# Neptune-Crypto/twenty-first

Hardware: AMD Instinct MI355X
Metric: goldilocks_ntt_gfelts_per_s (higher is better)
Workload: dtype u64

## Files before the change

### include/tf_hip.h

```cpp
#ifndef TF_HIP_H
#define TF_HIP_H

#include <stddef.h>
#include <stdint.h>

#ifdef __cplusplus
extern "C" {
#endif

enum tf_status {
    TF_OK = 0,
    TF_ERR_TOO_FEW_LEAFS = 1,
    TF_ERR_INCORRECT_NUMBER_OF_LEAFS = 2,
    TF_ERR_TREE_TOO_HIGH = 3,
    TF_ERR_LEN_NOT_POWER_OF_TWO = 4,
    TF_ERR_LEN_TOO_LARGE = 5,
    TF_ERR_ORDER_NOT_ABOVE_DEGREE = 6,
    TF_ERR_NULL_POINTER = 7,
    TF_ERR_NO_DEVICE = 8,
    TF_ERR_HIP = 9,
    TF_ERR_OUT_OF_MEMORY = 10,
    TF_ERR_LEAF_INDEX_INVALID = 11,
    TF_ERR_INVERSE_OF_ZERO = 12,
    TF_ERR_BUFFER_TOO_SMALL = 13,
// ... 199 lines not shown
int tf_tip5_sponge_sample_indices_dev(uint64_t *d_states, size_t count, uint32_t upper_bound, size_t num_indices, uint32_t *d_out_u32,
                                      void *stream);

int tf_batch_inversion_bfe(const uint64_t *in, size_t n, uint64_t *out);
int tf_batch_inversion_xfe(const uint64_t *in, size_t n, uint64_t *out);
int tf_batch_inversion_bfe_dev(const uint64_t *d_in, size_t n, uint64_t *d_out, void *stream);
int tf_batch_inversion_xfe_dev(const uint64_t *d_in, size_t n, uint64_t *d_out, void *stream);
int tf_batch_inversion_bfe_dev_async(const uint64_t *d_in, size_t n, uint64_t *d_out, void *stream, int *d_status);
int tf_batch_inversion_xfe_dev_async(const uint64_t *d_in, size_t n, uint64_t *d_out, void *stream, int *d_status);
int tf_inverse_or_zero_bfe(const uint64_t *in, size_t n, uint64_t *out);
int tf_inverse_or_zero_xfe(const uint64_t *in, size_t n, uint64_t *out);
int tf_inverse_or_zero_bfe_dev(const uint64_t *d_in, size_t n, uint64_t *d_out, void *stream);
int tf_inverse_or_zero_xfe_dev(const uint64_t *d_in, size_t n, uint64_t *d_out, void *stream);

void tf_set_ntt_tile_bytes(size_t bytes);
size_t tf_get_ntt_tile_bytes(void);
void tf_set_ntt_pipe(int streams);
int tf_get_ntt_pipe(void);

void tf_set_ntt_min_passes(int passes);
void tf_set_ntt_small_launch(int mode);
void tf_set_ntt_two_pass(int mode);
void tf_set_ntt_latency_kernel(int mode);
int tf_ntt_launch_count(size_t n, size_t batch, int width);
int tf_ntt_plan(size_t n, int width, int* log2_radix_out);
double tf_debug_sclk_mhz(void);

#ifdef TF_AB_BUILD
void tf_set_ntt_nt(int mask);
void tf_set_ntt_chain(int tiles_per_workgroup);
int tf_debug_stamps(unsigned long long *host_out, size_t words);
#endif
int tf_debug_fill_random_dev(uint64_t *d_out, size_t count, uint64_t seed, uint64_t first_index, void *stream);

#ifdef __cplusplus
}
#endif
#endif
```

### twenty-first_amd/_lib.py

```python
from __future__ import annotations

import ctypes as C
import os
import subprocess

_HERE = os.path.dirname(os.path.abspath(__file__))
SO_PATH = os.environ.get("TF_HIP_LIBRARY") or os.path.join(_HERE, "libtf_hip.so")
HEADER = os.path.join(os.path.dirname(_HERE), "include", "tf_hip.h")

_u64p = C.POINTER(C.c_uint64)
_sz = C.c_size_t
_vp = C.c_void_p

SIGNATURES = {
    "tf_status_string": (C.c_char_p, [C.c_int]),
    "tf_last_error": (C.c_char_p, []),
    "tf_version": (C.c_int, []),
    "tf_source_hash": (C.c_char_p, []),
    "tf_device_count": (C.c_int, []),
    "tf_set_device": (C.c_int, [C.c_int]),
    "tf_get_device": (C.c_int, [C.POINTER(C.c_int)]),
    "tf_shard_range": (C.c_int, [_sz, C.c_int, C.c_int, C.POINTER(_sz), C.POINTER(_sz)]),
    "tf_merkle_multi_subtrees": (C.c_int, [_sz, _sz, C.c_int]),
    "tf_prepare_ntt": (C.c_int, [_sz, _sz, C.c_int, C.c_int]),
# ... 130 lines not shown
    "tf_tip5_sponge_pad_and_absorb_all_dev": (C.c_int, [_vp, _sz, _vp, _sz, _vp, _vp]),
    "tf_tip5_sponge_squeeze": (C.c_int, [_vp, _sz, _sz, _vp]),
    "tf_tip5_sponge_squeeze_dev": (C.c_int, [_vp, _sz, _sz, _vp, _vp]),
    "tf_tip5_sponge_sample_scalars": (C.c_int, [_vp, _sz, _sz, _vp]),
    "tf_tip5_sponge_sample_scalars_dev": (C.c_int, [_vp, _sz, _sz, _vp, _vp]),
    "tf_tip5_sponge_sample_indices": (C.c_int, [_vp, _sz, C.c_uint32, _sz, _vp]),
    "tf_tip5_sponge_sample_indices_dev": (C.c_int, [_vp, _sz, C.c_uint32, _sz, _vp, _vp]),
    "tf_merkle_verify_proofs": (C.c_int, [_vp, _sz, _vp, _vp, _vp, _vp, _vp, _vp, _vp]),
    "tf_merkle_verify_proofs_dev": (C.c_int, [_vp, _sz, _vp, _vp, _vp, _vp, _vp, _vp, _vp, _vp]),
    "tf_merkle_authentication_paths": (C.c_int, [_vp, _sz, _vp, _vp, _vp, _vp, _vp, _vp, _vp]),
    "tf_merkle_authentication_paths_dev": (C.c_int, [_vp, _sz, _vp, _vp, _vp, _vp, _vp, _vp, _vp, _vp]),
    "tf_ntt_launch_count": (C.c_int, [_sz, _sz, C.c_int]),
    "tf_ntt_plan": (C.c_int, [_sz, C.c_int, C.POINTER(C.c_int)]),
    "tf_batch_eval_plan": (C.c_int, [_sz, _sz, _sz, C.c_int]),
    "tf_poly_interpolate_bfe_dev_async": (C.c_int, [_vp, _vp, _sz, _sz, _vp, _vp, _vp]),
    "tf_poly_interpolate_xfe_dev_async": (C.c_int, [_vp, _vp, _sz, _sz, _vp, _vp, _vp]),
    "tf_poly_clean_divide_bfe_dev_async": (C.c_int, [_vp, _sz, _vp, _sz, _vp, _vp, _vp]),
    "tf_poly_clean_divide_many_bfe_dev_async": (C.c_int, [_vp, _sz, _sz, _vp, _sz, _vp, _vp, _vp]),
    "tf_zerofier_tree_new_bfe_dev_async": (C.c_int, [_vp, _sz, _vp, C.POINTER(C.c_void_p)]),
    "tf_zerofier_tree_new_xfe_dev_async": (C.c_int, [_vp, _sz, _vp, C.POINTER(C.c_void_p)]),
    "tf_zerofier_tree_interpolate_dev_async": (C.c_int, [_vp, _vp, _sz, _vp, _vp, _vp]),
    "tf_release_caches": (C.c_int, []),
    "tf_set_ntt_small_launch": (None, [C.c_int]),
    "tf_set_ntt_two_pass": (None, [C.c_int]),
    "tf_set_ntt_latency_kernel": (None, [C.c_int]),
    "tf_debug_sclk_mhz": (C.c_double, []),
    "tf_set_ntt_tile_bytes": (None, [_sz]),
    "tf_set_ntt_min_passes": (None, [C.c_int]),
    "tf_get_ntt_tile_bytes": (_sz, []),
    "tf_set_ntt_pipe": (None, [C.c_int]),
    "tf_get_ntt_pipe": (C.c_int, []),
    "tf_set_batch_eval_route": (None, [C.c_int]),
    "tf_debug_fill_random_dev": (C.c_int, [_vp, _sz, C.c_uint64, C.c_uint64, _vp]),
}


AB_SIGNATURES = {
    "tf_set_ntt_chain": (None, [C.c_int]),
    "tf_debug_stamps": (C.c_int, [_vp, _sz]),
    "tf_set_ntt_nt": (None, [C.c_int]),
}


def build(force: bool = False) -> str:
    csrc = os.path.join(_HERE, "csrc")
    args = ["make", "-C", csrc]
    if force:
        args.append("-B")
    args.append(f"-j{min(8, os.cpu_count() or 1)}")
    subprocess.check_call(args, stdout=subprocess.DEVNULL)
    return SO_PATH


_lib = None


def _load_hip_runtime() -> None:
    candidates = []
    try:
        import torch

        candidates.append(os.path.join(os.path.dirname(torch.__file__), "lib", "libamdhip64.so"))
    except Exception:
        pass
    candidates += ["/opt/rocm/lib/libamdhip64.so", "libamdhip64.so"]
    errors = []
# ... 38 lines not shown
```

### twenty-first_amd/csrc/aux_kernels.h

```cpp
#pragma once

#include "gl64.h"

namespace tfk {

using gl::u32;
using gl::u64;

__global__ void sclk_probe_kernel(unsigned long long* out) {
    const unsigned long long w0 = wall_clock64(), c0 = clock64();
    unsigned v = threadIdx.x;
    for (int i = 0; i < 200000; ++i) v = v * 1664525u + 1013904223u;
    const unsigned long long c1 = clock64(), w1 = wall_clock64();
    if (threadIdx.x == 0) {
        out[0] = c1 - c0 + (v == 0xdeadbeefu);
        out[1] = w1 - w0;
    }
}

__global__ void __launch_bounds__(256) fill_random_kernel(u64* out, unsigned long long count, u64 seed, unsigned long long first) {
    const unsigned long long stride = (unsigned long long)gridDim.x * blockDim.x;
    for (unsigned long long i = (unsigned long long)blockIdx.x * blockDim.x + threadIdx.x; i < count; i += stride) {
        u64 z = (seed ^ (first + i)) + 0x9e3779b97f4a7c15ULL;
        z = (z ^ (z >> 30)) * 0xbf58476d1ce4e5b9ULL;
        z = (z ^ (z >> 27)) * 0x94d049bb133111ebULL;
        z ^= z >> 31;
        if (z >= gl::P) z -= gl::P;
        out[i] = gl::mont_mul(z, gl::R2);
    }
}

}
```

### twenty-first_amd/csrc/gl64.h

```cpp
#pragma once

#include <stdint.h>

#if defined(__HIPCC__)
#include <hip/hip_runtime.h>
#define GL_HD __host__ __device__ __forceinline__
#else
#define GL_HD inline
#endif

namespace gl {

typedef uint64_t u64;
typedef uint32_t u32;

constexpr u64 P = 0xffffffff00000001ULL;
constexpr u64 EPS = 0xffffffffULL;
constexpr u64 R2 = 0xfffffffe00000001ULL;
constexpr u64 ONE = 0xffffffffULL;

GL_HD u64 add(u64 a, u64 b) {
    u64 s = a + b;
    bool c = s < a;
    u64 t = s + EPS;
// ... 416 lines not shown
    static_assert(K > 0 && K < 32, "");
    const u64 lo = x << K;
    const u32 hi = (u32)(x >> (64 - K));
    const u64 t = (u64)hi * 0xffffffffu + lo;
    const bool c = t < lo;
    const u64 u = t + EPS;
    const bool c2 = u < t;
    return (c | c2) ? u : t;
}

template <int S>
GL_HD u64 shl_monty(u64 x) {
    static_assert(S >= 0 && S < 64, "");
#if defined(__HIP_DEVICE_COMPILE__)
    const u32 x0 = (u32)x, x1 = (u32)(x >> 32);
    u32 l0, l1, h0, h1;
    if constexpr (S == 0) {
        l0 = x0, l1 = x1, h0 = 0, h1 = 0;
    } else if constexpr (S < 32) {
        l0 = x0 << S, l1 = __builtin_amdgcn_alignbit(x1, x0, 32 - S), h0 = x1 >> (32 - S), h1 = 0;
    } else if constexpr (S == 32) {
        l0 = 0, l1 = x0, h0 = x1, h1 = 0;
    } else {
        l0 = 0, l1 = x0 << (S - 32), h0 = __builtin_amdgcn_alignbit(x1, x0, 64 - S), h1 = x1 >> (64 - S);
    }
    return montyred(((u64)l1 << 32) | l0, ((u64)h1 << 32) | h0);
#else
    const u64 lo = x << S;
    const u64 hi = S ? (x >> ((64 - S) & 63)) : 0;
    return montyred(lo, hi);
#endif
}

template <int E>
struct Pow2Mul {
    static constexpr int e96 = ((E % 192) + 192) % 192 % 96;
    static constexpr bool high = (((E % 192) + 192) % 192) >= 96;
    static constexpr bool via_monty = e96 >= 32;
    static constexpr bool negate = high != via_monty;
    static GL_HD u64 apply(u64 x) {
        if constexpr (e96 == 0) {
            return x;
        } else if constexpr (e96 < 32) {
            return shl_fold<e96>(x);
        } else {
            return shl_monty<e96 - 32>(x);
        }
    }
};

template <int K>
GL_HD u64 mul_pow2(u64 x) {
    const u64 v = Pow2Mul<K>::apply(x);
    if constexpr (Pow2Mul<K>::negate) return neg(v);
    return v;
}

}
```

### twenty-first_amd/csrc/ntt_kernels.h

```cpp
#pragma once

#include <type_traits>

#include "gl64.h"
#include "ntt_args.h"
#include "ntt_network.h"

namespace tfk {

using gl::u32;
using gl::u64;

struct NttPassArgs {
    const u64* in;
    u64* out;
    const u64* inner_tw;
    const u64* post_tw;
    const u64* pre_scale;
    long long n_out;
    const u64* in2;
    const u64* post_scale;
    long long js_i0, js_i1, js_i2, js_c, js_k;
    long long n_coeffs;
    long long ps_i1;
// ... 1093 lines not shown
            for (int i = 0; i < 8; ++i) wb[i] = tw_load(8 + i);
        }
        mul_store(0, wa);
#pragma unroll
        for (int i = 0; i < 8; ++i) wa[i] = tw_load(16 + i);
        __builtin_amdgcn_sched_barrier(0);
        mul_store(8, wb);
#pragma unroll
        for (int i = 0; i < 8; ++i) wb[i] = tw_load(24 + i);
        __builtin_amdgcn_sched_barrier(0);
        mul_store(16, wa);
        __builtin_amdgcn_sched_barrier(0);
        mul_store(24, wb);
    }
}

struct NttBlockArgs {
    const u64* in;
    u64* out;
    const u64* tw1;
    const u64* tw2;
    const u64* pre_scale;
    const u64* post_scale;
    long long n_coeffs;
    long long in_bs, out_bs;
    long long total_transforms;
    const u64* in2;
    long long n_out;
    int L;
};

template <int LOGP3, bool INV, int SCALE = 0>
__global__ void __launch_bounds__(512, 4) ntt_block_kernel(const NttBlockArgs A) {
    constexpr int P3 = 1 << LOGP3, N = 1024 << LOGP3, REST = 32 << LOGP3, T = 16 >> LOGP3;
    constexpr int PS1 = 1056 + 32 / P3;
    constexpr int KS2 = 32 * P3 + 1;
    extern __shared__ __attribute__((aligned(16))) u64 lds[];
    const int t = threadIdx.x;
    const long long tr0 = (long long)blockIdx.x * T;
    const int nt = (int)min((long long)T, A.total_transforms - tr0);
    u64 x[32];
    const int trA = t / REST, rest = t - trA * REST;
    const bool actA = trA < nt;
    const int es = A.L;
    {
        const long long ltA = tr0 + trA, slA = ltA / es;
        const u64* src = A.in + slA * A.in_bs + (ltA - slA * es) + (long long)rest * es;
        const long long lim = (SCALE != 1 || A.n_coeffs < 0) ? (long long)N : A.n_coeffs;
#pragma unroll
        for (int q = 0; q < 32; ++q) x[q] = (actA && (SCALE != 1 || brev5(q) * REST + rest < lim)) ? src[(long long)brev5(q) * REST * es] : 0;
        if (SCALE == 3) {
            const u64* src2 = A.in2 + (tr0 + trA) * A.in_bs + rest;
#pragma unroll
            for (int q0 = 0; q0 < 32; q0 += 8) {
                u64 w[8];
#pragma unroll
                for (int i = 0; i < 8; ++i) w[i] = actA ? src2[(long long)brev5(q0 + i) * REST] : 0;
#pragma unroll
                for (int i = 0; i < 8; i += 4) mul4_inplace(x, q0 + i, w[i], w[i + 1], w[i + 2], w[i + 3]);
            }
        }
        if (SCALE == 1 && A.pre_scale) {
            const u64* ps = A.pre_scale + rest;
#pragma unroll
            for (int q0 = 0; q0 < 32; q0 += 8) {
                u64 w[8];
#pragma unroll
                for (int i = 0; i < 8; ++i) {
                    const long long j = brev5(q0 + i) * REST + rest;
                    w[i] = ps[j < lim ? brev5(q0 + i) * REST : -rest];
                }
#pragma unroll
                for (int i = 0; i < 8; i += 4) mul4_inplace(x, q0 + i, w[i], w[i + 1], w[i + 2], w[i + 3]);
            }
        }
    }
    dit_half<INV, 0, true>(x);
    dit_half<INV, 16, true>(x);
    dit_level<INV, 5, true>(x);
    {
        const u64* tw = A.tw1 + rest;
#pragma unroll
        for (int q = 4; q < 32; q += 4) mul4_inplace(x, q, tw[q * REST], tw[(q + 1) * REST], tw[(q + 2) * REST], tw[(q + 3) * REST]);
        gl::mont_mul2(x[2], tw[2 * REST], x[3], tw[3 * REST], x[2], x[3]);
        x[1] = gl::mont_mul(x[1], tw[REST]);
#if TF_LAZY
        x[0] = gl::add(x[0], 0);
#endif
    }
    const int j2A = rest >> LOGP3, j3A = rest & (P3 - 1);
    const int pairA = trA * P3 + j3A;
    const int tb = (LOGP3 == 4) ? ((t & ~0x108) | ((t & 8) << 5) | ((t >> 5) & 8)) : t;
    const int trB = tb / REST, j3B = (tb >> 5) & (P3 - 1), k1B = tb & 31;
    const int pairB = trB * P3 + j3B;
#pragma unroll 1
    for (int r = 0; r < 2; ++r) {
        if (r) __syncthreads();
        if ((pairA >> 3) == r) {
            u64* wr = lds + (pairA & 7) * PS1 + j2A;
#pragma unroll
            for (int q = 0; q < 32; ++q) wr[q * 33] = x[q];
        }
        __syncthreads();
        if ((pairB >> 3) == r) {
            const u64* rd = lds + (pairB & 7) * PS1 + k1B * 33;
#pragma unroll
            for (int q = 0; q < 32; ++q) x[q] = rd[brev5(q)];
        }
    }
    dit_half<INV, 0, true>(x);
    dit_half<INV, 16, true>(x);
    dit_level<INV, 5, true>(x);
    {
        const u64* tw = A.tw2 + j3B;
#pragma unroll
        for (int q = 0; q < 32; q += 4) mul4_inplace(x, q, tw[q * P3], tw[(q + 1) * P3], tw[(q + 2) * P3], tw[(q + 3) * P3]);
    }
    const int trC = trB, sC = j3B, k1C = k1B;
    __syncthreads();
#pragma unroll 1
    for (int r = 0; r < 2; ++r) {
        if (r) __syncthreads();
        if ((k1B >> 4) == r) {
            u64* wr = lds + (trB * 16 + (k1B & 15)) * KS2 + j3B;
#pragma unroll
            for (int q = 0; q < 32; ++q) wr[q * P3] = x[q];
        }
        __syncthreads();
        if ((k1C >> 4) == r) {
            const u64* rd = lds + (trC * 16 + (k1C & 15)) * KS2 + sC * (32 / P3) * P3;
#pragma unroll
            for (int q = 0; q < 32; ++q) {
                const int grp = q >> LOGP3, rr = q & (P3 - 1);
                const int j3 = (int)(__brev((unsigned)rr) >> (32 - LOGP3));
                x[q] = rd[grp * P3 + j3];
            }
        }
    }
    if constexpr (LOGP3 >= 1) dit_level<INV, 1>(x);
    if constexpr (LOGP3 >= 2) dit_level<INV, 2>(x);
    if constexpr (LOGP3 >= 3) dit_level<INV, 3>(x);
    if constexpr (LOGP3 >= 4) dit_level<INV, 4>(x);
    if (trC < nt) {
        const long long ltC = tr0 + trC, slC = ltC / es;
        u64* dst = A.out + slC * A.out_bs + (ltC - slC * es) + (long long)k1C * es;
// ... 329 lines not shown
```

### twenty-first_amd/csrc/ntt_network.h

```cpp
#pragma once

#include "gl64.h"

namespace tfk {

using gl::u32;
using gl::u64;

template <bool INV, int LVL, int J>
struct TwExp {
    static constexpr int fwd = ((39 << (6 - LVL)) * J) % 192;
    static constexpr int value = INV ? (192 - fwd) % 192 : fwd;
};

#ifndef TF_ASM_BFLY
#define TF_ASM_BFLY 1
#endif
#ifndef TF_LDS_TW
#define TF_LDS_TW 1
#endif
constexpr int kLdsTwStride = 34;
constexpr int kR1024Nc = 16, kR1024Cpr = 8, kR1024Rounds = 2, kR1024S1 = 264;
constexpr int kL1024S1 = 273, kL1024CS = 34;
constexpr int kL1024ExchangeWords = ((31 * kL1024S1 + 7 * kL1024CS + 32 + 1) / 2) * 2;
#ifndef TF_LAZY
#define TF_LAZY 1
#endif

template <bool INV, int LVL, int I>
struct Bf {
    static constexpr int H = 1 << (LVL - 1);
    static constexpr int j = I % H;
    static constexpr int ia = (I / H) * 2 * H + j;
    static constexpr int ib = ia + H;
    static constexpr int E = TwExp<INV, LVL, j>::value;
    static constexpr bool neg = gl::Pow2Mul<E>::negate;
};

template <int E, bool LAZY_IN>
__device__ __forceinline__ u64 tw_operand(u64 b) {
    if constexpr (E % 192 == 0) {
        if constexpr (LAZY_IN) return gl::add(b, 0);
        return b;
    } else {
        return gl::Pow2Mul<E>::apply(b);
    }
}

template <bool INV, int LVL, int I, bool LAZY>
__device__ __forceinline__ void butterfly_pair(u64 (&x)[32]) {
    using B0 = Bf<INV, LVL, I>;
    using B1 = Bf<INV, LVL, I + 1>;
    const u64 v0 = tw_operand<B0::E, LAZY && (LVL > 1)>(x[B0::ib]);
    const u64 v1 = tw_operand<B1::E, LAZY && (LVL > 1)>(x[B1::ib]);
    u64 s0, d0, s1, d1;
    if constexpr (LAZY) gl::add_sub_lazy2(x[B0::ia], v0, x[B1::ia], v1, s0, d0, s1, d1);
    else gl::add_sub2(x[B0::ia], v0, x[B1::ia], v1, s0, d0, s1, d1);
    x[B0::ia] = B0::neg ? d0 : s0;
    x[B0::ib] = B0::neg ? s0 : d0;
    x[B1::ia] = B1::neg ? d1 : s1;
    x[B1::ib] = B1::neg ? s1 : d1;
}

template <int E>
__device__ __forceinline__ void butterfly_pow2(u64& a, u64& b) {
    const u64 v = gl::Pow2Mul<E>::apply(b);
#if TF_ASM_BFLY
    if constexpr (!gl::Pow2Mul<E>::negate) gl::add_sub(a, v, a, b);
    else gl::add_sub(a, v, b, a);
    return;
#endif
    if constexpr (!gl::Pow2Mul<E>::negate) {
        const u64 s = gl::add(a, v);
        b = gl::sub(a, v);
        a = s;
    } else {
        const u64 s = gl::sub(a, v);
        b = gl::add(a, v);
        a = s;
    }
}

template <bool INV, int LVL, int I, int END, bool LAZY>
struct DitRange {
    static __device__ __forceinline__ void run(u64 (&x)[32]) {
#if TF_ASM_BFLY
        butterfly_pair<INV, LVL, I, LAZY>(x);
#else
        butterfly_pow2<Bf<INV, LVL, I>::E>(x[Bf<INV, LVL, I>::ia], x[Bf<INV, LVL, I>::ib]);
        butterfly_pow2<Bf<INV, LVL, I + 1>::E>(x[Bf<INV, LVL, I + 1>::ia], x[Bf<INV, LVL, I + 1>::ib]);
#endif
        if constexpr (I + 2 < END) DitRange<INV, LVL, I + 2, END, LAZY>::run(x);
    }
};
template <bool INV, int LVL, bool LAZY = false>
__device__ __forceinline__ void dit_level(u64 (&x)[32]) { DitRange<INV, LVL, 0, 16, LAZY && TF_LAZY>::run(x); }

template <bool INV, int FIRST, bool LAZY = false>
__device__ __forceinline__ void dit_half(u64 (&x)[32]) {
    DitRange<INV, 1, FIRST / 2, FIRST / 2 + 8, LAZY && TF_LAZY>::run(x);
    DitRange<INV, 2, FIRST / 2, FIRST / 2 + 8, LAZY && TF_LAZY>::run(x);
    DitRange<INV, 3, FIRST / 2, FIRST / 2 + 8, LAZY && TF_LAZY>::run(x);
    DitRange<INV, 4, FIRST / 2, FIRST / 2 + 8, LAZY && TF_LAZY>::run(x);
}

__device__ __forceinline__ void mul4_inplace(u64 (&x)[32], int q0, u64 w0, u64 w1, u64 w2, u64 w3) {
    const u64 a4[4] = {x[q0], x[q0 + 1], x[q0 + 2], x[q0 + 3]}, b4[4] = {w0, w1, w2, w3};
    u64 r4[4];
    gl::mont_mul4(a4, b4, r4);
    x[q0] = r4[0], x[q0 + 1] = r4[1], x[q0 + 2] = r4[2], x[q0 + 3] = r4[3];
}

}
```

### twenty-first_amd/csrc/tf_abi.hip

```cpp
#include "tf_internal.h"
#include "aux_kernels.h"

#include <functional>

namespace tfi {

struct DevBuf {
    u64* p = nullptr;
    hipStream_t s;
    explicit DevBuf(hipStream_t st) : s(st) {}
    int alloc(size_t words) {
        if (words == 0) return TF_OK;
        hipError_t e = pool_malloc_async(reinterpret_cast<void**>(&p), words * sizeof(u64), s);
        if (e != hipSuccess) return hip_fail(e, "hipMallocAsync", __FILE__, __LINE__);
        return TF_OK;
    }
    ~DevBuf() {
        if (p) (void)hipFreeAsync(p, s);
    }
};

int h2d(u64* d, const u64* h, size_t words, hipStream_t s) {
    if (!words) return TF_OK;
    HIPCHK(hipMemcpyAsync(d, h, words * sizeof(u64), hipMemcpyHostToDevice, s));
    HIPCHK(hipStreamSynchronize(s));
    return TF_OK;
}

struct HostStreams {
    hipStream_t s[kMaxDevices] = {};
    ~HostStreams() {
        for (int d = 0; d < kMaxDevices; ++d)
            if (s[d]) (void)hipStreamDestroy(s[d]);
    }
};
hipStream_t host_stream() {
// ... 71 lines not shown
int merkle_proofs_host(const uint32_t* heights, size_t n, const uint64_t* loff, const uint64_t* idx, const uint64_t* dig, const uint64_t* aoff,
                       const uint64_t* auth, const uint64_t* roots, int* statuses, uint64_t* paths_out, bool paths) {
    if (n == 0) return TF_OK;
    if (!heights || !loff || !aoff || !statuses) return TF_ERR_NULL_POINTER;
    size_t path_words = 0;
    for (size_t p = 0; p < n; ++p) {
        if (loff[p + 1] < loff[p] || aoff[p + 1] < aoff[p]) return TF_ERR_INVALID_ARGUMENT;
        if (heights[p] < 64) path_words += (loff[p + 1] - loff[p]) * heights[p];
    }
    const size_t nk = loff[n] - loff[0], na = aoff[n] - aoff[0];
    if ((nk && (!idx || !dig)) || (na && !auth) || (!paths && !roots) || (paths && path_words && !paths_out)) return TF_ERR_NULL_POINTER;
    DeviceCtx* ctx = nullptr;
    TRY(current_ctx(&ctx));
    hipStream_t s = host_stream();
    DevBuf di(s), dd(s), da(s), dr(s), dst(s), dp(s);
    TRY(di.alloc(nk));
    TRY(dd.alloc(5 * nk));
    TRY(da.alloc(5 * na));
    TRY(dr.alloc(paths ? 0 : 5 * n));
    TRY(dst.alloc((n + 1) / 2));
    TRY(dp.alloc(paths ? 5 * path_words : 0));
    if (nk) {
        TRY(h2d(di.p, idx + loff[0], nk, s));
        TRY(h2d(dd.p, dig + 5 * loff[0], 5 * nk, s));
    }
    if (na) TRY(h2d(da.p, auth + 5 * aoff[0], 5 * na, s));
    if (!paths) TRY(h2d(dr.p, roots, 5 * n, s));
    TRY(merkle_proofs_dev(heights, n, loff, di.p, dd.p, aoff, da.p, dr.p, reinterpret_cast<int*>(dst.p), dp.p, paths, loff[0], aoff[0], s));
    HIPCHK(hipMemcpyAsync(statuses, dst.p, n * sizeof(int), hipMemcpyDeviceToHost, s));
    if (paths) TRY(d2h(paths_out, dp.p, 5 * path_words, s));
    return sync(s);
}

}

using namespace tfi;


extern "C" {

const char* tf_status_string(int status) {
    switch (status) {
        case TF_OK: return "TF_OK";
        case TF_ERR_TOO_FEW_LEAFS: return "TF_ERR_TOO_FEW_LEAFS";
        case TF_ERR_INCORRECT_NUMBER_OF_LEAFS: return "TF_ERR_INCORRECT_NUMBER_OF_LEAFS";
        case TF_ERR_TREE_TOO_HIGH: return "TF_ERR_TREE_TOO_HIGH";
        case TF_ERR_LEN_NOT_POWER_OF_TWO: return "TF_ERR_LEN_NOT_POWER_OF_TWO";
        case TF_ERR_LEN_TOO_LARGE: return "TF_ERR_LEN_TOO_LARGE";
        case TF_ERR_ORDER_NOT_ABOVE_DEGREE: return "TF_ERR_ORDER_NOT_ABOVE_DEGREE";
        case TF_ERR_NULL_POINTER: return "TF_ERR_NULL_POINTER";
        case TF_ERR_NO_DEVICE: return "TF_ERR_NO_DEVICE";
        case TF_ERR_HIP: return "TF_ERR_HIP";
        case TF_ERR_OUT_OF_MEMORY: return "TF_ERR_OUT_OF_MEMORY";
        case TF_ERR_LEAF_INDEX_INVALID: return "TF_ERR_LEAF_INDEX_INVALID";
        case TF_ERR_INVERSE_OF_ZERO: return "TF_ERR_INVERSE_OF_ZERO";
        case TF_ERR_BUFFER_TOO_SMALL: return "TF_ERR_BUFFER_TOO_SMALL";
        case TF_ERR_EMPTY_DOMAIN: return "TF_ERR_EMPTY_DOMAIN";
        case TF_ERR_DIVISION_BY_ZERO: return "TF_ERR_DIVISION_BY_ZERO";
        case TF_ERR_DIVISION_NOT_CLEAN: return "TF_ERR_DIVISION_NOT_CLEAN";
        case TF_ERR_INVALID_ARGUMENT: return "TF_ERR_INVALID_ARGUMENT";
        case TF_ERR_INTERNAL: return "TF_ERR_INTERNAL";
        case TF_ERR_AUTH_STRUCTURE_LENGTH_MISMATCH: return "TF_ERR_AUTH_STRUCTURE_LENGTH_MISMATCH";
        case TF_ERR_REPEATED_LEAF_DIGEST_MISMATCH: return "TF_ERR_REPEATED_LEAF_DIGEST_MISMATCH";
        case TF_ERR_ROOT_MISMATCH: return "TF_ERR_ROOT_MISMATCH";
        case TF_ERR_MMR_LEAF_INDEX_OUT_OF_RANGE: return "TF_ERR_MMR_LEAF_INDEX_OUT_OF_RANGE";
        case TF_ERR_MMR_PEAK_COUNT_MISMATCH: return "TF_ERR_MMR_PEAK_COUNT_MISMATCH";
// ... 48 lines not shown
}
int tf_get_ntt_pipe(void) {
    read_env();
    return g_pipe.load(std::memory_order_relaxed);
}

double tf_debug_sclk_mhz(void) {
    int dev = 0, wall_khz = 0;
    if (hipGetDevice(&dev) != hipSuccess) return -1.0;
    if (hipDeviceGetAttribute(&wall_khz, hipDeviceAttributeWallClockRate, dev) != hipSuccess || wall_khz <= 0) wall_khz = 100000;
    unsigned long long* d = nullptr;
    if (hipMalloc(reinterpret_cast<void**>(&d), 2 * sizeof(unsigned long long)) != hipSuccess) return -1.0;
    hipLaunchKernelGGL(tfk::sclk_probe_kernel, dim3(1), dim3(64), 0, hipStream_t(0), d);
    unsigned long long h[2] = {0, 0};
    const hipError_t e = hipMemcpy(h, d, sizeof(h), hipMemcpyDeviceToHost);
    (void)hipFree(d);
    if (e != hipSuccess || h[1] == 0) return -1.0;
    return (double)h[0] / (double)h[1] * (double)wall_khz / 1000.0;
}

int tf_debug_fill_random_dev(uint64_t* d_out, size_t count, uint64_t seed, uint64_t first_index, void* stream) try {
    if (count == 0) return TF_OK;
    if (!d_out) return TF_ERR_NULL_POINTER;
    DeviceCtx* ctx = nullptr;
    int rc = current_ctx(&ctx);
    if (rc) return rc;
    const unsigned blocks = (unsigned)std::min<size_t>((count + 255) / 256, size_t(1) << 20);
    hipLaunchKernelGGL(tfk::fill_random_kernel, dim3(blocks), dim3(256), 0, static_cast<hipStream_t>(stream), d_out,
                       (unsigned long long)count, (u64)seed, (unsigned long long)first_index);
    HIPCHK(hipGetLastError());
    return TF_OK;
} TF_ABI_CATCH

#ifdef TF_AB_BUILD
int tf_debug_stamps(unsigned long long* host_out, size_t words) try {
    if (!g_dbg_buf) {
        if (hipMalloc(reinterpret_cast<void**>(&g_dbg_buf), 4096 * 8 * 6 * 8) != hipSuccess) return TF_ERR_HIP;
        (void)hipMemset(g_dbg_buf, 0, 4096 * 8 * 6 * 8);
    }
    if (host_out && words) {
        if (hipDeviceSynchronize() != hipSuccess) return TF_ERR_HIP;
        if (hipMemcpy(host_out, g_dbg_buf, std::min<size_t>(words, 4096 * 8 * 6) * 8, hipMemcpyDeviceToHost) != hipSuccess) return TF_ERR_HIP;
    }
    return TF_OK;
} TF_ABI_CATCH
#endif

void tf_set_ntt_min_passes(int passes) { g_min_passes.store(passes, std::memory_order_relaxed); }
#ifdef TF_AB_BUILD
void tf_set_ntt_chain(int tiles_per_workgroup) { g_chain.store(std::max(0, tiles_per_workgroup), std::memory_order_relaxed); }
#endif
void tf_set_ntt_latency_kernel(int mode) { g_lat_mode.store(mode < 0 ? -1 : (mode ? 1 : 0), std::memory_order_relaxed); }
void tf_set_ntt_two_pass(int mode) { g_pre2_mode.store(mode < 0 ? -1 : (mode > 3 ? 1 : mode), std::memory_order_relaxed); }
void tf_set_ntt_small_launch(int mode) { g_small_launch_mode.store(mode < 0 ? -1 : (mode ? 1 : 0), std::memory_order_relaxed); }
int tf_batch_eval_plan(size_t n_coeffs, size_t n_points, size_t batch, int width) {
    if (width != 1 && width != 3) return 0;
    return tree_route(n_coeffs, n_points, batch, width) ? 2 : 1;
}
int tf_ntt_plan(size_t n, int width, int* log2_radix_out) {
    if (check_len(n) || n <= 1 || (width != 1 && width != 3) || !log2_radix_out) return 0;
    const int log_n = ilog2(n);
    for (int i = 0; i < 4; ++i) log2_radix_out[i] = 0;
    static const bool no_block = ab_env("TF_NTT_NO_BLOCK") != nullptr;
    static const bool no_xfe_block = ab_env("TF_NTT_NO_XFE_BLOCK") != nullptr;
    if (log_n <= 10 || (log_n <= (width == 1 ? 14 : (no_xfe_block ? 10 : 12)) && !no_block && g_min_passes.load(std::memory_order_relaxed) == 0)) {
        log2_radix_out[0] = log_n;
// ... 776 lines not shown
```

### twenty-first_amd/device.py

```python
from __future__ import annotations

import ctypes as C

from . import _lib


def _chk(rc, where):
    from . import _check

    _check(rc, where)


def _t(t, name="tensor"):
    import torch

    if not isinstance(t, torch.Tensor) or not t.is_cuda or not t.is_contiguous() or t.dtype not in (torch.int64, torch.uint64):
        raise TypeError(f"{name} must be a contiguous CUDA int64/uint64 tensor of raw Montgomery words")
    return t


def _stream(stream):
    import torch

    s = stream if stream is not None else torch.cuda.current_stream()
    return C.c_void_p(s.cuda_stream)


def _p(t):
    return C.c_void_p(t.data_ptr())


def _need(cond: bool, what: str) -> None:
    if not cond:
        raise ValueError(what)


def _width(width: int) -> int:
    _need(width in (1, 3), "width must be 1 (BFieldElement) or 3 (XFieldElement)")
    return width


def fill_random(out, seed: int, first_index: int = 0, stream=None) -> None:
    out = _t(out, "out")
    _chk(_lib.lib().tf_debug_fill_random_dev(_p(out), out.numel(), C.c_uint64(seed & (2 ** 64 - 1)), C.c_uint64(first_index),
                                             _stream(stream)), "fill_random")


def ntt_(x, n: int, batch: int = 1, width: int = 1, inverse: bool = False, stream=None) -> None:
    x = _t(x, "x")
    _width(width)
    if x.numel() != n * batch * width:
        raise ValueError("tensor size is not batch * n * width")
    fn = _lib.lib().tf_ntt_bfe_dev if width == 1 else _lib.lib().tf_ntt_xfe_dev
    _chk(fn(_p(x), n, batch, int(inverse), _stream(stream)), "intt" if inverse else "ntt")


def coset_evaluate(coeffs, n_coeffs: int, offset_raw: int, out, order: int, batch: int = 1, width: int = 1, stream=None) -> None:
    coeffs, out = _t(coeffs, "coeffs"), _t(out, "out")
    _width(width)
    if coeffs.numel() != n_coeffs * batch * width or out.numel() != order * batch * width:
        raise ValueError("buffer sizes do not match n_coeffs/order/batch/width")
    fn = _lib.lib().tf_coset_eval_bfe_dev if width == 1 else _lib.lib().tf_coset_eval_xfe_dev
    _chk(fn(_p(coeffs), n_coeffs, C.c_uint64(offset_raw), _p(out), order, batch, _stream(stream)), "fast_coset_evaluate")


def tip5_permute_(states, stream=None) -> None:
    states = _t(states, "states")
    _need(states.numel() % 16 == 0, "states must hold 16 words per Tip5 state")
    _chk(_lib.lib().tf_tip5_permute_dev(_p(states), states.numel() // 16, _stream(stream)), "Tip5::permutation")


def tip5_trace_(states, trace, stream=None) -> None:
    states, trace = _t(states, "states"), _t(trace, "trace")
    _need(states.numel() % 16 == 0 and trace.numel() == 6 * states.numel(), "trace must hold 6 x 16 words per Tip5 state")
    _chk(_lib.lib().tf_tip5_trace_dev(_p(states), _p(trace), states.numel() // 16, _stream(stream)), "Tip5::trace")


def tip5_hash_pairs(inp, out, stream=None) -> None:
# ... 496 lines not shown
```

Baseline: 146.0.

## Group power-of-two twiddle butterflies by class and use inline asm reduction

Adds hand-written GCN inline assembly for the shift-and-reduce multiplications by powers of two in Goldilocks, batched 2 or 4 wide so independent carry chains interleave without nops. The radix-32 butterfly network now reorders butterflies within a level by exponent class so same-class twiddles can share one asm block. The aim is to cut VALU instruction count and dependency stalls in the block NTT kernel. It also adds a debug kernel and ABI entry to test mul_pow2. The risks are register pressure, and inline asm that may block compiler scheduling or hide a subtle carry bug.

```diff
diff --git a/include/tf_hip.h b/include/tf_hip.h
--- a/include/tf_hip.h
+++ b/include/tf_hip.h
@@ -255,6 +255,7 @@
 int tf_debug_stamps(unsigned long long *host_out, size_t words);
 #endif
 int tf_debug_fill_random_dev(uint64_t *d_out, size_t count, uint64_t seed, uint64_t first_index, void *stream);
+int tf_debug_mul_pow2_dev(uint64_t *d_x, size_t count, int e, void *stream);
 
 #ifdef __cplusplus
 }
diff --git a/twenty-first_amd/_lib.py b/twenty-first_amd/_lib.py
--- a/twenty-first_amd/_lib.py
+++ b/twenty-first_amd/_lib.py
@@ -186,6 +186,7 @@
     "tf_get_ntt_pipe": (C.c_int, []),
     "tf_set_batch_eval_route": (None, [C.c_int]),
     "tf_debug_fill_random_dev": (C.c_int, [_vp, _sz, C.c_uint64, C.c_uint64, _vp]),
+    "tf_debug_mul_pow2_dev": (C.c_int, [_vp, _sz, C.c_int, _vp]),
 }
 
 
diff --git a/twenty-first_amd/csrc/aux_kernels.h b/twenty-first_amd/csrc/aux_kernels.h
--- a/twenty-first_amd/csrc/aux_kernels.h
+++ b/twenty-first_amd/csrc/aux_kernels.h
@@ -30,4 +30,29 @@
     }
 }
 
+template <int E>
+__global__ void __launch_bounds__(256) mul_pow2_kernel(u64* x, unsigned long long count) {
+    const unsigned long long base = ((unsigned long long)blockIdx.x * blockDim.x + threadIdx.x) * 6;
+    u64 v4[4], v2[2];
+#pragma unroll
+    for (int i = 0; i < 4; ++i) v4[i] = base + i < count ? x[base + i] : 0;
+#pragma unroll
+    for (int i = 0; i < 2; ++i) v2[i] = base + 4 + i < count ? x[base + 4 + i] : 0;
+    if constexpr (gl::Pow2Mul<E>::cls == 0) {
+#pragma unroll
+        for (int i = 0; i < 4; ++i) v4[i] = gl::add(v4[i], 0);
+#pragma unroll
+        for (int i = 0; i < 2; ++i) v2[i] = gl::add(v2[i], 0);
+    } else {
+        gl::pow2_mul_block<E, E, E, E>(v4);
+        gl::pow2_mul_block<E, E>(v2);
+    }
+#pragma unroll
+    for (int i = 0; i < 4; ++i)
+        if (base + i < count) x[base + i] = gl::Pow2Mul<E>::negate ? gl::neg(v4[i]) : v4[i];
+#pragma unroll
+    for (int i = 0; i < 2; ++i)
+        if (base + 4 + i < count) x[base + 4 + i] = gl::Pow2Mul<E>::negate ? gl::neg(v2[i]) : v2[i];
 }
+
+}
diff --git a/twenty-first_amd/csrc/gl64.h b/twenty-first_amd/csrc/gl64.h
--- a/twenty-first_amd/csrc/gl64.h
+++ b/twenty-first_amd/csrc/gl64.h
@@ -472,22 +472,151 @@
 #endif
 }
 
+#ifndef TF_ASM_POW2
+#define TF_ASM_POW2 1
+#endif
+
+#if defined(__HIPCC__)
+template <int K>
+__device__ __forceinline__ u64 shl_fold_asm(u64 x) {
+    static_assert(K > 0 && K < 32, "");
+    const u64 lo = x << K;
+    const u32 hi = (u32)(x >> 32) >> (32 - K);
+    u64 t, c, ge, n;
+    asm("v_mad_u64_u32 %0, %1, %2, -1, %3" : "=v"(t), "=s"(c) : "v"(hi), "v"(lo));
+    u32 r0, r1;
+    asm("v_cmp_lt_u64_e64 %[ge], %[pm1], %[t]\n\t"
+        "s_or_b64 %[c], %[c], %[ge]\n\t"
+        "v_subbrev_co_u32_e64 %[r0], %[n], 0, %[t0], %[c]\n\t"
+        "s_andn2_b64 %[c], %[c], %[n]\n\t"
+        "v_addc_co_u32_e64 %[r1], %[n], 0, %[t1], %[c]"
+        : [r0] "=&v"(r0), [r1] "=v"(r1), [c] "+s"(c), [n] "=&s"(n), [ge] "=&s"(ge)
+        : [pm1] "s"(P - 1), [t] "v"(t), [t0] "v"((u32)t), [t1] "v"((u32)(t >> 32))
+        : "scc");
+    return ((u64)r1 << 32) | r0;
+}
+
+__device__ __forceinline__ u64 canonical_asm(u64 x) {
+    u32 r0, r1;
+    u64 c, n;
+    asm("v_cmp_lt_u64_e64 %[n], %[pm1], %[x]\n\t"
+        "s_mov_b64 %[c], %[n]\n\t"
+        "v_subbrev_co_u32_e64 %[r0], %[n], 0, %[x0], %[c]\n\t"
+        "s_andn2_b64 %[c], %[c], %[n]\n\t"
+        "v_addc_co_u32_e64 %[r1], %[n], 0, %[x1], %[c]"
+        : [r0] "=&v"(r0), [r1] "=v"(r1), [c] "=&s"(c), [n] "=&s"(n)
+        : [pm1] "s"(P - 1), [x] "v"(x), [x0] "v"((u32)x), [x1] "v"((u32)(x >> 32))
+        : "scc");
+    return ((u64)r1 << 32) | r0;
+}
+
+#define TF_P2_RR1(S) S(a)
+#define TF_P2_RR2(S) S(a) S(b)
+#define TF_P2_RR4(S) S(a) S(b) S(c) S(d)
+#define TF_P2_GAP1 "s_nop 1\n\t"
+#define TF_P2_GAP2 "s_nop 0\n\t"
+#define TF_P2_GAP4
+#define TF_P2B_1(X) "v_add_co_u32_e64 %[u" #X "], %[c" #X "], %[u" #X "], %[w" #X "]\n\t"
+#define TF_P2B_2(X) "v_subb_co_u32_e64 %[w" #X "], %[c" #X "], %[w" #X "], %[u" #X "], %[c" #X "]\n\t"
+#define TF_P2B_3(X) "v_subbrev_co_u32_e64 %[u" #X "], %[c" #X "], 0, %[u" #X "], %[c" #X "]\n\t"
+#define TF_P2B_4(X) "v_sub_co_u32_e64 %[r" #X "], %[c" #X "], %[r" #X "], %[w" #X "]\n\t"
+#define TF_P2B_5(X) "v_subb_co_u32_e64 %[u" #X "], %[c" #X "], 0, %[u" #X "], %[c" #X "]\n\t"
+#define TF_P2B_6(X) "v_addc_co_u32_e64 %[r" #X "], %[k" #X "], 0, %[r" #X "], %[c" #X "]\n\t"
+#define TF_P2B_7(X) "s_andn2_b64 %[c" #X "], %[c" #X "], %[k" #X "]\n\t"
+#define TF_P2B_8(X) "v_subbrev_co_u32_e64 %[u" #X "], %[k" #X "], 0, %[u" #X "], %[c" #X "]\n\t"
+#define TF_P2B_BODY(RR, GAP) RR(TF_P2B_1) GAP RR(TF_P2B_2) GAP RR(TF_P2B_3) RR(TF_P2B_4) GAP RR(TF_P2B_5) GAP RR(TF_P2B_6) RR(TF_P2B_7) RR(TF_P2B_8)
+#define TF_P2B_OPS(X, i) [w##X] "+v"(w[i]), [u##X] "+v"(u[i]), [r##X] "+v"(r[i]), [c##X] "=&s"(c[i]), [k##X] "=&s"(k[i])
+#define TF_P2C_1(X) "v_sub_co_u32_e64 %[w" #X "], %[c" #X "], 0, %[u" #X "]\n\t"
+#define TF_P2C_2(X) "v_subbrev_co_u32_e64 %[u" #X "], %[c" #X "], 0, %[u" #X "], %[c" #X "]\n\t"
+#define TF_P2C_3(X) "v_sub_co_u32_e64 %[r" #X "], %[c" #X "], %[r" #X "], %[w" #X "]\n\t"
+#define TF_P2C_4(X) "v_subb_co_u32_e64 %[q" #X "], %[c" #X "], %[q" #X "], %[u" #X "], %[c" #X "]\n\t"
+#define TF_P2C_5(X) "v_addc_co_u32_e64 %[r" #X "], %[k" #X "], 0, %[r" #X "], %[c" #X "]\n\t"
+#define TF_P2C_6(X) "s_andn2_b64 %[c" #X "], %[c" #X "], %[k" #X "]\n\t"
+#define TF_P2C_7(X) "v_subbrev_co_u32_e64 %[q" #X "], %[k" #X "], 0, %[q" #X "], %[c" #X "]\n\t"
+#define TF_P2C_BODY(RR, GAP) RR(TF_P2C_1) GAP RR(TF_P2C_2) RR(TF_P2C_3) GAP RR(TF_P2C_4) GAP RR(TF_P2C_5) RR(TF_P2C_6) RR(TF_P2C_7)
+#define TF_P2C_OPS(X, i) [w##X] "=&v"(w[i]), [u##X] "+v"(u[i]), [r##X] "+v"(r[i]), [q##X] "+v"(q[i]), [c##X] "=&s"(c[i]), [k##X] "=&s"(k[i])
+
+template <bool HIGH, int N>
+__device__ __forceinline__ void shl_monty_block(u64 (&x)[N], const int (&S)[N]) {
+    static_assert(N == 1 || N == 2 || N == 4, "");
+    u32 w[N], u[N], r[N], q[N];
+    u64 c[N], k[N];
+#pragma unroll
+    for (int i = 0; i < N; ++i) {
+        const int T = S[i] & 31;
+        const u32 x0 = (u32)x[i], x1 = (u32)(x[i] >> 32);
+        const u32 v0 = x0 << T, v1 = T ? __builtin_amdgcn_alignbit(x1, x0, 32 - T) : x1, v2 = T ? x1 >> (32 - T) : 0u;
+        if constexpr (HIGH) u[i] = v0, r[i] = v1, q[i] = v2;
+        else w[i] = v0, u[i] = v1, r[i] = v2;
+    }
+    if constexpr (!HIGH) {
+        if constexpr (N == 1) asm(TF_P2B_BODY(TF_P2_RR1, TF_P2_GAP1) : TF_P2B_OPS(a, 0) : : "scc");
+        else if constexpr (N == 2) asm(TF_P2B_BODY(TF_P2_RR2, TF_P2_GAP2) : TF_P2B_OPS(a, 0), TF_P2B_OPS(b, 1) : : "scc");
+        else asm(TF_P2B_BODY(TF_P2_RR4, TF_P2_GAP4) : TF_P2B_OPS(a, 0), TF_P2B_OPS(b, 1), TF_P2B_OPS(c, 2), TF_P2B_OPS(d, 3) : : "scc");
+#pragma unroll
+        for (int i = 0; i < N; ++i) x[i] = ((u64)u[i] << 32) | r[i];
+    } else {
+        if constexpr (N == 1) asm(TF_P2C_BODY(TF_P2_RR1, TF_P2_GAP1) : TF_P2C_OPS(a, 0) : : "scc");
+        else if constexpr (N == 2) asm(TF_P2C_BODY(TF_P2_RR2, TF_P2_GAP2) : TF_P2C_OPS(a, 0), TF_P2C_OPS(b, 1) : : "scc");
+        else asm(TF_P2C_BODY(TF_P2_RR4, TF_P2_GAP4) : TF_P2C_OPS(a, 0), TF_P2C_OPS(b, 1), TF_P2C_OPS(c, 2), TF_P2C_OPS(d, 3) : : "scc");
+#pragma unroll
+        for (int i = 0; i < N; ++i) x[i] = ((u64)q[i] << 32) | r[i];
+    }
+}
+#endif
+
+#if defined(__HIP_DEVICE_COMPILE__) && TF_ASM_POW2
+#define TF_POW2_DEVICE_ASM 1
+#else
+#define TF_POW2_DEVICE_ASM 0
+#endif
+
 template <int E>
 struct Pow2Mul {
     static constexpr int e96 = ((E % 192) + 192) % 192 % 96;
     static constexpr bool high = (((E % 192) + 192) % 192) >= 96;
     static constexpr bool via_monty = e96 >= 32;
     static constexpr bool negate = high != via_monty;
+    static constexpr int cls = e96 == 0 ? 0 : e96 < 32 ? 1 : e96 < 64 ? 2 : 3;
     static GL_HD u64 apply(u64 x) {
         if constexpr (e96 == 0) {
             return x;
         } else if constexpr (e96 < 32) {
+#if TF_POW2_DEVICE_ASM
+            return shl_fold_asm<e96>(x);
+#else
             return shl_fold<e96>(x);
+#endif
         } else {
+#if TF_POW2_DEVICE_ASM
+            u64 v[1] = {x};
+            const int s[1] = {e96 - 32};
+            shl_monty_block<(e96 >= 64), 1>(v, s);
+            return v[0];
+#else
             return shl_monty<e96 - 32>(x);
+#endif
         }
     }
 };
+
+#if defined(__HIPCC__)
+template <int... E>
+__device__ __forceinline__ void pow2_mul_block(u64 (&x)[sizeof...(E)]) {
+    constexpr int N = sizeof...(E);
+    constexpr int cls[N] = {Pow2Mul<E>::cls...};
+    static_assert(((Pow2Mul<E>::cls == cls[0]) && ...), "one exponent class per block");
+#if TF_POW2_DEVICE_ASM
+    if constexpr (cls[0] >= 2) {
+        const int s[N] = {(Pow2Mul<E>::e96 - 32)...};
+        shl_monty_block<(cls[0] == 3), N>(x, s);
+        return;
+    }
+#endif
+    int i = 0;
+    ((x[i] = Pow2Mul<E>::apply(x[i]), ++i), ...);
+}
+#endif
 
 template <int K>
 GL_HD u64 mul_pow2(u64 x) {
diff --git a/twenty-first_amd/csrc/ntt_kernels.h b/twenty-first_amd/csrc/ntt_kernels.h
--- a/twenty-first_amd/csrc/ntt_kernels.h
+++ b/twenty-first_amd/csrc/ntt_kernels.h
@@ -1149,6 +1149,7 @@
 
 template <int LOGP3, bool INV, int SCALE = 0>
 __global__ void __launch_bounds__(512, 4) ntt_block_kernel(const NttBlockArgs A) {
+    constexpr int W = LOGP3 == 4 ? 2 : TF_POW2_WIDE;
     constexpr int P3 = 1 << LOGP3, N = 1024 << LOGP3, REST = 32 << LOGP3, T = 16 >> LOGP3;
     constexpr int PS1 = 1056 + 32 / P3;
     constexpr int KS2 = 32 * P3 + 1;
@@ -1192,9 +1193,9 @@
             }
         }
     }
-    dit_half<INV, 0, true>(x);
-    dit_half<INV, 16, true>(x);
-    dit_level<INV, 5, true>(x);
+    dit_half<INV, 0, true, W>(x);
+    dit_half<INV, 16, true, W>(x);
+    dit_level<INV, 5, true, W>(x);
     {
         const u64* tw = A.tw1 + rest;
 #pragma unroll
@@ -1225,9 +1226,9 @@
             for (int q = 0; q < 32; ++q) x[q] = rd[brev5(q)];
         }
     }
-    dit_half<INV, 0, true>(x);
-    dit_half<INV, 16, true>(x);
-    dit_level<INV, 5, true>(x);
+    dit_half<INV, 0, true, W>(x);
+    dit_half<INV, 16, true, W>(x);
+    dit_level<INV, 5, true, W>(x);
     {
         const u64* tw = A.tw2 + j3B;
 #pragma unroll
diff --git a/twenty-first_amd/csrc/ntt_network.h b/twenty-first_amd/csrc/ntt_network.h
--- a/twenty-first_amd/csrc/ntt_network.h
+++ b/twenty-first_amd/csrc/ntt_network.h
@@ -40,6 +40,9 @@
 template <int E, bool LAZY_IN>
 __device__ __forceinline__ u64 tw_operand(u64 b) {
     if constexpr (E % 192 == 0) {
+#if TF_ASM_POW2
+        if constexpr (LAZY_IN) return gl::canonical_asm(b);
+#endif
         if constexpr (LAZY_IN) return gl::add(b, 0);
         return b;
     } else {
@@ -81,9 +84,99 @@
     }
 }
 
-template <bool INV, int LVL, int I, int END, bool LAZY>
+#ifndef TF_POW2_WIDE
+#define TF_POW2_WIDE 4
+#endif
+#if TF_ASM_BFLY && TF_ASM_POW2
+constexpr int bf_exp(bool inv, int lvl, int i) {
+    const int fwd = ((39 << (6 - lvl)) * (i % (1 << (lvl - 1)))) % 192;
+    return inv ? (192 - fwd) % 192 : fwd;
+}
+constexpr int bf_cls(bool inv, int lvl, int i) {
+    const int e96 = bf_exp(inv, lvl, i) % 96;
+    return e96 == 0 ? 0 : e96 < 32 ? 1 : e96 < 64 ? 2 : 3;
+}
+constexpr int bf_count(bool inv, int lvl, int i0, int end, int cls) {
+    int n = 0;
+    for (int i = i0; i < end; ++i) n += bf_cls(inv, lvl, i) == cls;
+    return n;
+}
+constexpr int bf_nth(bool inv, int lvl, int i0, int end, int cls, int pos) {
+    for (int i = i0; i < end; ++i)
+        if (bf_cls(inv, lvl, i) == cls && pos-- == 0) return i;
+    return i0;
+}
+template <typename BA, typename BB, bool LAZY>
+__device__ __forceinline__ void bfly2(u64 (&x)[32]) {
+    u64 s0, d0, s1, d1;
+    if constexpr (LAZY) gl::add_sub_lazy2(x[BA::ia], x[BA::ib], x[BB::ia], x[BB::ib], s0, d0, s1, d1);
+    else gl::add_sub2(x[BA::ia], x[BA::ib], x[BB::ia], x[BB::ib], s0, d0, s1, d1);
+    x[BA::ia] = BA::neg ? d0 : s0;
+    x[BA::ib] = BA::neg ? s0 : d0;
+    x[BB::ia] = BB::neg ? d1 : s1;
+    x[BB::ib] = BB::neg ? s1 : d1;
+}
+template <bool INV, int LVL, int I0, int END, int CLS, bool LAZY, int WIDE, int POS = 0>
+__device__ __forceinline__ void class_fused(u64 (&x)[32]) {
+    constexpr int rem = bf_count(INV, LVL, I0, END, CLS) - POS;
+    if constexpr (rem >= 2) {
+        constexpr int take = (rem >= 4 && WIDE >= 4) ? 4 : 2;
+        using A = Bf<INV, LVL, bf_nth(INV, LVL, I0, END, CLS, POS)>;
+        using B = Bf<INV, LVL, bf_nth(INV, LVL, I0, END, CLS, POS + 1)>;
+        using C = Bf<INV, LVL, bf_nth(INV, LVL, I0, END, CLS, POS + (take > 2 ? 2 : 0))>;
+        using D = Bf<INV, LVL, bf_nth(INV, LVL, I0, END, CLS, POS + (take > 2 ? 3 : 1))>;
+        if constexpr (CLS == 0) {
+            x[A::ib] = tw_operand<A::E, LAZY && (LVL > 1)>(x[A::ib]);
+            x[B::ib] = tw_operand<B::E, LAZY && (LVL > 1)>(x[B::ib]);
+            bfly2<A, B, LAZY>(x);
+        } else if constexpr (take == 2) {
+            u64 v[2] = {x[A::ib], x[B::ib]};
+            gl::pow2_mul_block<A::E, B::E>(v);
+            x[A::ib] = v[0], x[B::ib] = v[1];
+            bfly2<A, B, LAZY>(x);
+        } else {
+            u64 v[4] = {x[A::ib], x[B::ib], x[C::ib], x[D::ib]};
+            gl::pow2_mul_block<A::E, B::E, C::E, D::E>(v);
+            x[A::ib] = v[0], x[B::ib] = v[1], x[C::ib] = v[2], x[D::ib] = v[3];
+            bfly2<A, B, LAZY>(x);
+            bfly2<C, D, LAZY>(x);
+        }
+        class_fused<INV, LVL, I0, END, CLS, LAZY, WIDE, POS + (CLS == 0 ? 2 : take)>(x);
+    }
+}
+constexpr int bf_leftover(bool inv, int lvl, int i0, int end, int k) {
+    for (int c = 0; c < 4; ++c) {
+        const int n = bf_count(inv, lvl, i0, end, c);
+        if ((n & 1) && k-- == 0) return bf_nth(inv, lvl, i0, end, c, n - 1);
+    }
+    return -1;
+}
+template <bool INV, int LVL, int I0, int END, bool LAZY, int K = 0>
+__device__ __forceinline__ void leftover_fused(u64 (&x)[32]) {
+    constexpr int ia = bf_leftover(INV, LVL, I0, END, K), ib = bf_leftover(INV, LVL, I0, END, K + 1);
+    if constexpr (ia >= 0) {
+        static_assert(ib >= 0, "an even number of butterflies leaves an even number over");
+        using A = Bf<INV, LVL, ia>;
+        using B = Bf<INV, LVL, (ib >= 0 ? ib : 0)>;
+        x[A::ib] = tw_operand<A::E, LAZY && (LVL > 1)>(x[A::ib]);
+        x[B::ib] = tw_operand<B::E, LAZY && (LVL > 1)>(x[B::ib]);
+        bfly2<A, B, LAZY>(x);
+        leftover_fused<INV, LVL, I0, END, LAZY, K + 2>(x);
+    }
+}
+#endif
+
+template <bool INV, int LVL, int I, int END, bool LAZY, int WIDE = TF_POW2_WIDE>
 struct DitRange {
     static __device__ __forceinline__ void run(u64 (&x)[32]) {
+#if TF_ASM_BFLY && TF_ASM_POW2
+        static_assert(bf_exp(INV, LVL, I) == Bf<INV, LVL, I>::E && bf_exp(INV, LVL, END - 1) == Bf<INV, LVL, END - 1>::E, "");
+        class_fused<INV, LVL, I, END, 0, LAZY, WIDE>(x);
+        class_fused<INV, LVL, I, END, 1, LAZY, WIDE>(x);
+        class_fused<INV, LVL, I, END, 2, LAZY, WIDE>(x);
+        class_fused<INV, LVL, I, END, 3, LAZY, WIDE>(x);
+        leftover_fused<INV, LVL, I, END, LAZY>(x);
+#else
 #if TF_ASM_BFLY
         butterfly_pair<INV, LVL, I, LAZY>(x);
 #else
@@ -91,17 +184,18 @@
         butterfly_pow2<Bf<INV, LVL, I + 1>::E>(x[Bf<INV, LVL, I + 1>::ia], x[Bf<INV, LVL, I + 1>::ib]);
 #endif
         if constexpr (I + 2 < END) DitRange<INV, LVL, I + 2, END, LAZY>::run(x);
+#endif
     }
 };
-template <bool INV, int LVL, bool LAZY = false>
-__device__ __forceinline__ void dit_level(u64 (&x)[32]) { DitRange<INV, LVL, 0, 16, LAZY && TF_LAZY>::run(x); }
-
-template <bool INV, int FIRST, bool LAZY = false>
+template <bool INV, int LVL, bool LAZY = false, int WIDE = TF_POW2_WIDE>
+__device__ __forceinline__ void dit_level(u64 (&x)[32]) { DitRange<INV, LVL, 0, 16, LAZY && TF_LAZY, WIDE>::run(x); }
+
+template <bool INV, int FIRST, bool LAZY = false, int WIDE = TF_POW2_WIDE>
 __device__ __forceinline__ void dit_half(u64 (&x)[32]) {
-    DitRange<INV, 1, FIRST / 2, FIRST / 2 + 8, LAZY && TF_LAZY>::run(x);
-    DitRange<INV, 2, FIRST / 2, FIRST / 2 + 8, LAZY && TF_LAZY>::run(x);
-    DitRange<INV, 3, FIRST / 2, FIRST / 2 + 8, LAZY && TF_LAZY>::run(x);
-    DitRange<INV, 4, FIRST / 2, FIRST / 2 + 8, LAZY && TF_LAZY>::run(x);
+    DitRange<INV, 1, FIRST / 2, FIRST / 2 + 8, LAZY && TF_LAZY, WIDE>::run(x);
+    DitRange<INV, 2, FIRST / 2, FIRST / 2 + 8, LAZY && TF_LAZY, WIDE>::run(x);
+    DitRange<INV, 3, FIRST / 2, FIRST / 2 + 8, LAZY && TF_LAZY, WIDE>::run(x);
+    DitRange<INV, 4, FIRST / 2, FIRST / 2 + 8, LAZY && TF_LAZY, WIDE>::run(x);
 }
 
 __device__ __forceinline__ void mul4_inplace(u64 (&x)[32], int q0, u64 w0, u64 w1, u64 w2, u64 w3) {
diff --git a/twenty-first_amd/csrc/tf_abi.hip b/twenty-first_amd/csrc/tf_abi.hip
--- a/twenty-first_amd/csrc/tf_abi.hip
+++ b/twenty-first_amd/csrc/tf_abi.hip
@@ -2,6 +2,7 @@
 #include "aux_kernels.h"
 
 #include <functional>
+#include <utility>
 
 namespace tfi {
 
@@ -139,6 +140,17 @@
     return sync(s);
 }
 
+template <int E>
+void mul_pow2_launch(u64* d_x, size_t count, hipStream_t s) {
+    const unsigned blocks = (unsigned)((count + 6 * 256 - 1) / (6 * 256));
+    hipLaunchKernelGGL(tfk::mul_pow2_kernel<E>, dim3(blocks), dim3(256), 0, s, d_x, (unsigned long long)count);
+}
+template <int... E>
+void mul_pow2_dispatch(int e, u64* d_x, size_t count, hipStream_t s, std::integer_sequence<int, E...>) {
+    using Fn = void (*)(u64*, size_t, hipStream_t);
+    static const Fn table[] = {&mul_pow2_launch<E>...};
+    table[e](d_x, count, s);
+}
 }
 
 using namespace tfi;
@@ -253,6 +265,18 @@
     return TF_OK;
 } TF_ABI_CATCH
 
+int tf_debug_mul_pow2_dev(uint64_t* d_x, size_t count, int e, void* stream) try {
+    if (e < 0 || e >= 192 || count > (size_t(1) << 40)) return TF_ERR_INVALID_ARGUMENT;
+    if (count == 0) return TF_OK;
+    if (!d_x) return TF_ERR_NULL_POINTER;
+    DeviceCtx* ctx = nullptr;
+    int rc = current_ctx(&ctx);
+    if (rc) return rc;
+    mul_pow2_dispatch(e, reinterpret_cast<u64*>(d_x), count, static_cast<hipStream_t>(stream), std::make_integer_sequence<int, 192>{});
+    HIPCHK(hipGetLastError());
+    return TF_OK;
+} TF_ABI_CATCH
+
 #ifdef TF_AB_BUILD
 int tf_debug_stamps(unsigned long long* host_out, size_t words) try {
     if (!g_dbg_buf) {
diff --git a/twenty-first_amd/device.py b/twenty-first_amd/device.py
--- a/twenty-first_amd/device.py
+++ b/twenty-first_amd/device.py
@@ -44,6 +44,12 @@
     out = _t(out, "out")
     _chk(_lib.lib().tf_debug_fill_random_dev(_p(out), out.numel(), C.c_uint64(seed & (2 ** 64 - 1)), C.c_uint64(first_index),
                                              _stream(stream)), "fill_random")
+
+
+def debug_mul_pow2_(x, e: int, stream=None) -> None:
+    x = _t(x, "x")
+    _need(0 <= e < 192, "the exponent must be in [0, 192)")
+    _chk(_lib.lib().tf_debug_mul_pow2_dev(_p(x), x.numel(), int(e), _stream(stream)), "debug_mul_pow2")
 
 
 def ntt_(x, n: int, batch: int = 1, width: int = 1, inverse: bool = False, stream=None) -> None:
```

New measurement: 149.1, median of 6. 1.02x the previous value.
